# david-cortes/cmfrec

Measured on AMD Instinct MI355X. Metric: ALS rows/sec ((users+items)/iteration time), implicit ALS-CG k=50 fp64, higher is better.
Workload: dtype f64

## Files before the change

cmfrec_amd/csrc/cg_kernels.hpp:

```cpp
#pragma once
#include <hip/hip_runtime.h>
#include <stdint.h>
#include <type_traits>

#include "lanes.hpp"

namespace cmfhip {

constexpr int WAVE = 64;
constexpr int TILE = 64;
constexpr int MAX_W = 8;
#ifndef CMF_CG_WAVES_PER_SIMD
#define CMF_CG_WAVES_PER_SIMD 2
#endif
#ifndef CMF_CG_WAVES_PER_SIMD_F32
#define CMF_CG_WAVES_PER_SIMD_F32 3
#endif
#ifndef CMF_CG_WAVES_PER_SIMD_LOW
#define CMF_CG_WAVES_PER_SIMD_LOW 3
#endif
constexpr int CG_NTSEL_MAX_S = 7;
template <typename T, int W, int NRES_, int NTSEL = 0> constexpr int cg_waves_per_simd()
{
    if (sizeof(T) == 8 && NTSEL == 1 && W <= 8) return CMF_CG_WAVES_PER_SIMD_LOW;
    if (sizeof(T) == 4 && NTSEL == 1 && W <= 4 && NRES_ == 0) return CMF_CG_WAVES_PER_SIMD_F32 + 1;
    return (sizeof(T) == 4 && W <= 4 && NRES_ == 0) ? CMF_CG_WAVES_PER_SIMD_F32 : CMF_CG_WAVES_PER_SIMD;
}
constexpr int CG_NT_LOW = 6;
#ifndef CMF_CG_NT_F32
#define CMF_CG_NT_F32 1
#endif
#ifndef CMF_CG_NT_MIN_S
#define CMF_CG_NT_MIN_S 4
#endif

struct RowDesc {
    int row;
    int nnz;
    unsigned long long st;
};

constexpr int CG_NCOUNTERS = 64;
constexpr int CG_COUNTER_STRIDE = 32;

template <typename T>
__device__ __forceinline__ T cg_div(T num, T den)
{
#ifndef CMF_CG_IEEE_DIV
    if constexpr (sizeof(T) == 4) return num * __builtin_amdgcn_rcpf(den);
    else {
        double y = __builtin_amdgcn_rcp(den);
        double e = __builtin_fma(-den, y, 1.0);
        y = __builtin_fma(y, e, y);
        e = __builtin_fma(-den, y, 1.0);
        y = __builtin_fma(y, e, y);
        double q = num * y;
        const double r = __builtin_fma(-den, q, num);
        return __builtin_fma(r, y, q);
    }
#else
    return num / den;
#endif
}

template <typename V>
__device__ __forceinline__ V lds_g(const V *p) { return *p; }

template <typename T>
struct CgParams {
    T *A;
    size_t lda;
    const T *B;
    size_t ldb;
    int k;
    const size_t *indptr;
    const int *indices;
    const T *values;
    const T *bias_sub;
    const T *weights = nullptr;
    const T *wsum = nullptr;
    const int *order;
    const RowDesc *desc;
    int nrows;
    const T *BtB;
    T lam, lam_last;
    int scale_lam, scale_bias_const;
    int max_cg_steps;
    int precond;
    int koff = 0, kc = 0;
    const T *CtC = nullptr;
    const T *UC = nullptr;
    T w_side = 0;
    int rows_with_u = 0;
    int row_first = 0;
    const size_t *indptr2 = nullptr;
    const int *indices2 = nullptr;
    const T *values2 = nullptr;
    const T *C2 = nullptr;
    int *counter = nullptr;
    int p_side = 0, scale_lam_sideinfo = 0;
    const T *Bi = nullptr;
    const T *BiTBi = nullptr;
    int ki = 0;
    T w_imp = 0;
    const T *rconst = nullptr;
    size_t ldr = 0;
    int gx = 0;
#ifdef CMF_CG_DEBUG
    int dbg = 0;
#endif
#ifdef CMF_CG_TICKS
    unsigned long long *ticks = nullptr;
#endif
};
#ifdef CMF_CG_TICKS
#define CMF_TICK() __builtin_amdgcn_s_memtime()
__device__ __forceinline__ void cg_ticks_flush(unsigned long long *t, int slot, unsigned long long wait, unsigned long long pass, unsigned long long rows,
                                               unsigned long long total, int lane)
{
    if (t != nullptr && lane == 0) {
        atomicAdd(t + 4 * slot + 0, wait); atomicAdd(t + 4 * slot + 1, pass); atomicAdd(t + 4 * slot + 2, rows); atomicAdd(t + 4 * slot + 3, total);
    }
}
#endif
#ifdef CMF_CG_DEBUG
#define CMF_DBG(P, bit) (((P).dbg & (bit)) != 0)
#else
#define CMF_DBG(P, bit) false
#endif
template <int NT, int S, typename TILE, typename T>
__device__ __forceinline__ void dbg_fill_tile(TILE &tile, T val)
{
#pragma unroll
    for (int t = 0; t < NT; t++)
#pragma unroll
        for (int s = 0; s < S; s++) tile.set(t, s, val);
}

template <typename T>
__device__ __forceinline__ T wave_sum(T v) { return lanes::wave_sum(v); }

template <typename T, int NT, int I>
__device__ __forceinline__ T treduce8_low_first(const T (&v)[8], bool h)
{
    if constexpr (I + 4 < NT) {
        T keep = h ? v[I + 4] : v[I];
        return keep + lanes::recv_xor4(v[I], v[I + 4]);
    } else return v[I] + lanes::xor4_lower(v[I]);
}
template <typename T, int NT = 8>
__device__ __forceinline__ T treduce8_low(const T (&v)[8], int lane)
{
    static_assert(NT >= 4 && NT <= 8, "entries per lane group");
    T u[4], q[2];
    bool h = (lane & 4) != 0;
    u[0] = treduce8_low_first<T, NT, 0>(v, h); u[1] = treduce8_low_first<T, NT, 1>(v, h);
    u[2] = treduce8_low_first<T, NT, 2>(v, h); u[3] = treduce8_low_first<T, NT, 3>(v, h);
    h = (lane & 2) != 0;
#pragma unroll
    for (int i = 0; i < 2; i++) {
        T keep = h ? u[i + 2] : u[i];
        T send = h ? u[i] : u[i + 2];
        q[i] = keep + lanes::xor2(send);
    }
    h = (lane & 1) != 0;
    T keep = h ? q[1] : q[0];
    T send = h ? q[0] : q[1];
    return keep + lanes::xor1(send);
}

template <typename T>
__device__ __forceinline__ T treduce8_high(const T (&v)[8], int lane)
{
    T u[4], q[2];
#pragma unroll
    for (int i = 0; i < 4; i++) u[i] = lanes::tswap32_add(v[i], v[i + 4]);
#pragma unroll
    for (int i = 0; i < 2; i++) q[i] = lanes::tswap16_add(u[i], u[i + 2]);
    const bool h = (lane & 8) != 0;
    T keep = h ? q[1] : q[0];
    return keep + lanes::recv_xor8(q[0], q[1]);
}

#ifndef CMF_PASS_VECTOR_LDS
#define CMF_PASS_VECTOR_LDS 2
#endif
template <typename T> constexpr bool pass_vector_in_lds() { return CMF_PASS_VECTOR_LDS == 1 || (CMF_PASS_VECTOR_LDS == 2 && sizeof(T) == 8); }
template <typename T, int S>
__device__ __forceinline__ void replicate(T vdist, T (&vrep)[S], int lane);
template <typename T, int S, int GR = 8>
__device__ __forceinline__ void pass_vector_lds(T vdist, T (&vrep)[S], T (&wts)[8], int lane, T *__restrict__ pv)
{
    const int jj = lane >> 3, ll = lane & 7;
    pv[lane] = vdist;
    __builtin_amdgcn_wave_barrier();
#pragma unroll
    for (int s = 0; s < S; s++) vrep[s] = pv[ll + 8 * s];
    const T *wp = pv + GR * jj;
#pragma unroll
    for (int t = 0; t < GR; t++) wts[t] = wp[t];
    __builtin_amdgcn_wave_barrier();
}

__host__ __device__ constexpr int gram_ld(int S) { return 8 * S + 1; }
#ifndef CMF_GRAM_ROWS_BY_K
#define CMF_GRAM_ROWS_BY_K 1
#endif
template <typename T> __host__ __device__ constexpr int gram_rows(int S) { return (CMF_GRAM_ROWS_BY_K && pass_vector_in_lds<T>()) ? S : 8; }
__host__ __device__ constexpr int gram_ld_rows(int S, int GR)
{
    if (GR == 8) return gram_ld(S);
    int ld = 8 * S;
    while ((S * ld) % 32 != 8 && (S * ld) % 32 != 24) ld++;
    return ld;
}
__host__ __device__ constexpr int gram_ld2(int S) { return 8 * S + 2; }
template <typename T> __host__ __device__ constexpr int gram_elems(int S) { return sizeof(T) == 4 ? 64 * gram_ld2(S) : 64 * gram_ld(S); }
template <typename T, int S, int GR = 8> __device__ __forceinline__ int gram_index(int r, int c)
{
    if constexpr (sizeof(T) == 4) return 2 * ((r >> 1) * gram_ld2(S) + c) + (r & 1);
    else return r * gram_ld_rows(S, GR) + c;
}
template <typename T, int S, int GR = 8>
__device__ __forceinline__ void stage_gramian(T *__restrict__ G, const T *__restrict__ BtB, int k, int tid, int nthreads)
{
    static_assert(GR == 8 || sizeof(T) == 8, "rows by k: double precision");
    for (int e = tid; e < 8 * GR * 8 * S; e += nthreads) {
        const int r = e / (8 * S), c = e % (8 * S);
        G[gram_index<T, S, GR>(r, c)] = (r < k && c < k) ? BtB[(size_t)r * k + c] : T(0);
    }
}

template <typename T, int S>
struct RegTile {
    T v[8][S];
    __device__ __forceinline__ void set(int t, int s, T x) { v[t][s] = x; }
};
typedef float f32x2 __attribute__((ext_vector_type(2)));
template <int S>
struct RegTile<float, S> {
    f32x2 v[4][S];
    __device__ __forceinline__ void set(int t, int s, float x) { v[t >> 1][s][t & 1] = x; }
};

template <typename T>
struct PassAcc {
    T v[8];
    __device__ __forceinline__ void zero()
    {
#pragma unroll
        for (int s = 0; s < 8; s++) v[s] = T(0);
    }
    __device__ __forceinline__ void close(T (&out)[8]) const
    {
#pragma unroll
        for (int s = 0; s < 8; s++) out[s] = v[s];
    }
};
template <>
struct PassAcc<float> {
    f32x2 v[8];
    __device__ __forceinline__ void zero()
    {
#pragma unroll
        for (int s = 0; s < 8; s++) v[s] = f32x2{0.f, 0.f};
    }
    __device__ __forceinline__ void close(float (&out)[8]) const
    {
#pragma unroll
        for (int s = 0; s < 8; s++) out[s] = v[s][0] + v[s][1];
    }
};

#ifndef CMF_CG_EARLY_GATHER
#define CMF_CG_EARLY_GATHER 0
#endif
struct NoAfter {
    template <typename TAG> __device__ __forceinline__ void operator()(TAG) const {}
};
template <int S, typename ACC>
__device__ __forceinline__ void pin_acc(ACC &out)
{
#pragma unroll
    for (int s = 0; s < S; s++) asm volatile("" : "+v"(out.v[s]));
}
template <int TS, typename T, int S, typename TILE>
__device__ __forceinline__ void load_tile_slot(TILE &tile, const char *base, unsigned ldb_bytes, unsigned it, int col_last)
{
    const T *rp = reinterpret_cast<const T *>(base + (unsigned long long)it * ldb_bytes);
#pragma unroll
    for (int s = 0; s < S; s++) tile.set(TS, s, rp[(s < S - 1) ? 8 * s : col_last]);
}

template <typename T, int S, int NT = 8>
__device__ __forceinline__ void load_tile(RegTile<T, S> &tile, const T *__restrict__ Bm, size_t ldb,
                                          int k, int my_idx, int cnt, int lane)
{
    const int jj = lane >> 3, ll = lane & 7;
    int its[8];
    its[0] = lanes::bcast8<0>(my_idx); its[1] = lanes::bcast8<1>(my_idx); its[2] = lanes::bcast8<2>(my_idx);
    its[3] = lanes::bcast8<3>(my_idx);
    if (NT > 4) its[4] = lanes::bcast8<4>(my_idx);
    if (NT > 5) its[5] = lanes::bcast8<5>(my_idx);
    if (NT > 6) its[6] = lanes::bcast8<6>(my_idx);
    if (NT > 7) its[7] = lanes::bcast8<7>(my_idx);
    const int first_idx = __builtin_amdgcn_readfirstlane(my_idx);
    const int col_last = min(ll + 8 * (S - 1), k - 1) - ll;
    const char *base = reinterpret_cast<const char *>(Bm + ll);
    const unsigned ldb_bytes = (unsigned)(ldb * sizeof(T));
#pragma unroll
    for (int t = 0; t < NT; t++) {
        const unsigned it = (unsigned)(((jj * NT + t) < cnt) ? its[t] : first_idx);
        const T *rp = reinterpret_cast<const T *>(base + (unsigned long long)it * ldb_bytes);
#pragma unroll
        for (int s = 0; s < S; s++) tile.set(t, s, rp[(s < S - 1) ? 8 * s : col_last]);
    }
}

template <typename T, bool IMPLICIT, int MODE>
__device__ __forceinline__ T pass_weight(T coef, T x, bool valid, T g = T(1))
{
    T w;
    if (IMPLICIT) {
        if (MODE == 0) w = -(coef - T(1)) * x - coef;
        else           w = coef * (x - T(1)) + coef;
    } else {
        if (MODE == 0) w = -((coef - x) * g);
        else           w = coef * g;
    }
    return valid ? w : T(0);
}

template <typename T>
__device__ __forceinline__ T row_lam_mult(const CgParams<T> &P, int row, int nnz)
{
    return (P.wsum != nullptr) ? P.wsum[row] : (T)nnz;
}
template <typename T, bool IMPLICIT>
__device__ __forceinline__ T entry_weight(const CgParams<T> &P, size_t pos)
{
    if (IMPLICIT) return T(1);
    return (P.weights != nullptr) ? P.weights[pos] : T(1);
}

template <int S, bool IMPLICIT, int MODE, int NT = 8, bool INIT = false, typename AFTER = NoAfter>
__device__ __forceinline__ void tile_pass_f32(const RegTile<float, S> &tile, const float (&vrep)[S], float x, bool valid,
                                          PassAcc<float> &out, int lane, float g = 1.f, AFTER after = AFTER())
{
    static_assert(NT % 2 == 0, "single precision: the entries of a lane group travel in pairs");
    float c[8];
#pragma unroll
    for (int q = 0; q < NT / 2; q++) {
        f32x2 acc = f32x2{0.f, 0.f};
#pragma unroll
        for (int s = 0; s < S; s++) acc += tile.v[q][s] * f32x2{vrep[s], vrep[s]};
        c[2 * q] = acc[0]; c[2 * q + 1] = acc[1];
    }
    float coef = treduce8_low<float, NT>(c, lane);
    const float w = pass_weight<float, IMPLICIT, MODE>(coef, x, valid, g);
    float wts[8];
    wts[0] = lanes::bcast8<0>(w); wts[1] = lanes::bcast8<1>(w); wts[2] = lanes::bcast8<2>(w); wts[3] = lanes::bcast8<3>(w);
    if (NT > 4) { wts[4] = lanes::bcast8<4>(w); wts[5] = lanes::bcast8<5>(w); }
    if (NT > 6) { wts[6] = lanes::bcast8<6>(w); wts[7] = lanes::bcast8<7>(w); }
    if constexpr (std::is_same<AFTER, NoAfter>::value) {
#pragma unroll
    for (int q = 0; q < NT / 2; q++) {
        const f32x2 w2 = f32x2{wts[2 * q], wts[2 * q + 1]};
#pragma unroll
        for (int s = 0; s < S; s++) out.v[s] = (INIT && q == 0) ? w2 * tile.v[q][s] : out.v[s] + w2 * tile.v[q][s];
    }
    } else {
        static_for<0, NT / 2>([&](auto qc) {
            constexpr int q = decltype(qc)::value;
            const f32x2 w2 = f32x2{wts[2 * q], wts[2 * q + 1]};
#pragma unroll
            for (int s = 0; s < S; s++) out.v[s] = (INIT && q == 0) ? w2 * tile.v[q][s] : out.v[s] + w2 * tile.v[q][s];
            pin_acc<S>(out);
            after(std::integral_constant<int, 2 * q>{});
            after(std::integral_constant<int, 2 * q + 1>{});
        });
    }
    if constexpr (INIT) {
#pragma unroll
        for (int s = S; s < 8; s++) out.v[s] = f32x2{0.f, 0.f};
    }
}

template <typename T, int S, bool IMPLICIT, int MODE, int NT = 8, bool INIT = false, typename AFTER = NoAfter>
__device__ __forceinline__ void tile_pass(const RegTile<T, S> &tile, const T (&vrep)[S], T x, bool valid,
                                          PassAcc<T> &out, int lane, T g = T(1), AFTER after = AFTER())
{
    if constexpr (std::is_same<T, float>::value) {
        tile_pass_f32<S, IMPLICIT, MODE, NT, INIT, AFTER>(tile, vrep, x, valid, out, lane, g, after);
    } else {
    T c[8];
// ... 71 lines not shown
    constexpr int LD = gram_ld_rows(S, GR);
    const int jj = lane >> 3, ll = lane & 7;
    if constexpr (std::is_same<T, float>::value && W <= 4) {
#pragma unroll
        for (int q = 0; q < 4; q++) {
            if (W > 1 && (q % W) != wr) continue;
            const f32x2 *g = reinterpret_cast<const f32x2 *>(G) + (jj * 4 + q) * gram_ld2(S) + ll;
            const f32x2 w2 = f32x2{wts[2 * q], wts[2 * q + 1]};
#pragma unroll
            for (int s = 0; s < S; s++) out.v[s] = NEG ? out.v[s] - w2 * lds_g(g + 8 * s) : out.v[s] + w2 * lds_g(g + 8 * s);
        }
    } else {
#pragma unroll
        for (int t = 0; t < GR; t++) {
            if (W > 1 && (t % W) != wr) continue;
#pragma unroll
            for (int s = 0; s < S; s++) {
                if constexpr (std::is_same<T, float>::value) {
                    const float g = G[gram_index<T, S>(jj * 8 + t, ll + 8 * s)];
                    out.v[s][0] = NEG ? out.v[s][0] - wts[t] * g : out.v[s][0] + wts[t] * g;
                } else {
                    const T g = lds_g(G + (jj * GR + t) * LD + ll + 8 * s);
                    out.v[s] = NEG ? out.v[s] - wts[t] * g : out.v[s] + wts[t] * g;
                }
            }
        }
    }
}

template <typename T, int S>
__device__ __forceinline__ void replicate(T vdist, T (&vrep)[S], int lane)
{
    const int ll = lane & 7;
#pragma unroll
    for (int s = 0; s < S; s++) vrep[s] = __shfl(vdist, s * 8 + ll);
}

template <typename T, int S, bool IMPLICIT, int W, int RPB, bool GRAMX = false, int NRES_ = 0, int NTSEL = 0>
__global__ void __launch_bounds__(64 * W * RPB, (cg_waves_per_simd<T, W, NRES_, NTSEL>()))
cg_rows_kernel(const CgParams<T> P)
{
    constexpr bool GRAM = IMPLICIT || GRAMX;
    extern __shared__ __attribute__((aligned(16))) unsigned char smem_raw[];
    T *G = reinterpret_cast<T *>(smem_raw);
    T *red = G + (GRAM ? gram_elems<T>(S) : 0);
    const int tid = threadIdx.x;
    const int lane = tid & 63;
    const int wave = tid >> 6;
    const int grp = wave / W;
    const int wr = wave % W;
    const int k = P.k;

    const int nteams = gridDim.x * RPB;
    __shared__ int s_claim[4];
    constexpr bool PV = pass_vector_in_lds<T>();
    __shared__ __attribute__((aligned(16))) T s_pv[PV ? W * RPB : 1][PV ? 64 : 1];
    const int cslot = (blockIdx.x * RPB + grp) % CG_NCOUNTERS;
    int *const my_counter = P.counter + cslot * CG_COUNTER_STRIDE;
    const int cbase = nteams + cslot;
    auto issue_claim = [&]() -> int {
        int v = 0;
        if (wr == 0 && lane == 0) v = atomicAdd(my_counter, 1);
        return v;
    };
    int rnxt, rnn;
    if (W == 1) {
        const int c1 = issue_claim(), c2 = issue_claim();
        rnxt = cbase + CG_NCOUNTERS * __builtin_amdgcn_readfirstlane(c1);
        rnn = cbase + CG_NCOUNTERS * __builtin_amdgcn_readfirstlane(c2);
    } else if (wr == 0 && lane == 0) {
        s_claim[2] = cbase + CG_NCOUNTERS * atomicAdd(my_counter, 1);
        s_claim[3] = cbase + CG_NCOUNTERS * atomicAdd(my_counter, 1);
    }
    constexpr int GR = gram_rows<T>(S);
    if (GRAM) stage_gramian<T, S, GR>(G, P.BtB, k, tid, blockDim.x);
    if (GRAM || W > 1) __syncthreads();
    if (W > 1) { rnxt = s_claim[2]; rnn = s_claim[3]; }
    T *myred = red + (size_t)grp * 2 * W * 64;

    int buf = 0;
    static_assert(W == 1 || RPB == 1, "multi-wave teams own their workgroup (barriers are per row)");

    constexpr int NRES = NRES_ > 0 ? NRES_ : ((std::is_same<T, float>::value && W == 8) ? 2 : 1);
    static_assert(NRES == 1 || std::is_same<T, float>::value, "two resident tiles: single precision");
    static_assert(NTSEL == 0 || (S >= CMF_CG_NT_MIN_S && (sizeof(T) == 4 || S <= CG_NTSEL_MAX_S) && NRES_ == 0),
                  "launches by tile size: tiles by row length (double precision: k <= 56)");
    constexpr int NT_MIN = (S >= CMF_CG_NT_MIN_S && (CMF_CG_NT_F32 || !std::is_same<T, float>::value)) ? (std::is_same<T, float>::value ? 6 : 5) : 8;
    auto nt_of = [&](int nnz_) -> int {
        int nt = (nnz_ + 8 * W * NRES - 1) / (8 * W * NRES);
        if (std::is_same<T, float>::value) nt = (nt + 1) & ~1;
        return (nt > 8) ? 8 : (nt < NT_MIN ? NT_MIN : nt);
    };
    struct Pre { int idx; T x; T a; int idx2; T x2; T g; T g2; };
    auto load_desc = [&](int rix_) -> RowDesc {
        RowDesc d; d.row = 0; d.nnz = 0; d.st = 0;
        if (rix_ < P.nrows) d = P.desc[rix_];
        d.row = __builtin_amdgcn_readfirstlane(d.row);
        d.nnz = __builtin_amdgcn_readfirstlane(d.nnz);
        d.st = ((unsigned long long)(unsigned)__builtin_amdgcn_readfirstlane((int)(d.st >> 32)) << 32) |
               (unsigned)__builtin_amdgcn_readfirstlane((int)(d.st & 0xffffffffu));
        return d;
    };
    auto load_pre = [&](const RowDesc &d) -> Pre {
        Pre q; q.idx = 0; q.x = T(0); q.a = T(0); q.idx2 = 0; q.x2 = T(0); q.g = T(1); q.g2 = T(1);
        const int nt = nt_of(d.nnz), tl = 8 * nt;
        const int b = lane & 7;
        const int ent = (lane >> 3) * nt + b;
        const int cnt = min(tl, d.nnz - wr * tl);
        if (b < nt && ent < cnt) {
            const size_t pos = d.st + (size_t)wr * tl + ent;
            q.idx = P.indices[pos];
            q.x = P.values[pos];
            q.g = entry_weight<T, IMPLICIT>(P, pos);
            if (!IMPLICIT && P.bias_sub != nullptr) q.x -= P.bias_sub[q.idx];
        }
        if (NRES == 2) {
            const int cnt2 = min(tl, d.nnz - (wr + W) * tl);
            if (b < nt && ent < cnt2) {
                const size_t pos = d.st + (size_t)(wr + W) * tl + ent;
                q.idx2 = P.indices[pos];
                q.x2 = P.values[pos];
                q.g2 = entry_weight<T, IMPLICIT>(P, pos);
                if (!IMPLICIT && P.bias_sub != nullptr) q.x2 -= P.bias_sub[q.idx2];
            }
        }
        if (d.nnz > 0 && lane < k) q.a = P.A[(size_t)d.row * P.lda + lane];
        return q;
    };
    int rix = blockIdx.x * RPB + grp;
    RowDesc dcur = load_desc(rix);
    RowDesc dnxt = load_desc(rnxt);
    Pre pcur = load_pre(dcur);
    int pend = issue_claim();
    constexpr bool EARLY = CMF_CG_EARLY_GATHER != 0;
    constexpr int NT_MAX = (NTSEL == 1) ? CG_NT_LOW : 8;
    RegTile<T, S> tile_c;
    RegTile<T, (NRES == 2) ? S : 1> tile2_c;
    const char *const gbase = reinterpret_cast<const char *>(P.B + (lane & 7));
    const unsigned gldb = (unsigned)(P.ldb * sizeof(T));
    const int gcol_last = min((lane & 7) + 8 * (S - 1), k - 1) - (lane & 7);
    auto gather_slot = [&](auto &tl_, auto tc, int idx_, int first_idx_, int nt_, int cnt_) {
        constexpr int t = decltype(tc)::value;
        if constexpr (t < NT_MAX) {
            if (t < nt_) {
                const unsigned it_ = (unsigned)((((lane >> 3) * nt_ + t) < cnt_) ? lanes::bcast8<t>(idx_) : first_idx_);
                load_tile_slot<t, T, S>(tl_, gbase, gldb, it_, gcol_last);
            }
        }
    };
    struct Want { int nt0, cnt0, nt1, cnt1; };
    auto want_of = [&](const RowDesc &d) -> Want {
        Want w_;
        const int nt = nt_of(d.nnz), tl = 8 * nt;
        w_.cnt0 = min(tl, d.nnz - wr * tl);
        w_.nt0 = (w_.cnt0 > 0 && !CMF_DBG(P, 1)) ? nt : 0;
        w_.cnt1 = (NRES == 2) ? min(tl, d.nnz - (wr + W) * tl) : 0;
        w_.nt1 = (w_.cnt1 > 0 && !CMF_DBG(P, 1)) ? nt : 0;
        return w_;
    };
    auto gather_row = [&](const RowDesc &d, const Pre &q) {
        const Want w_ = want_of(d);
        const int f0 = __builtin_amdgcn_readfirstlane(q.idx);
        static_for<0, NT_MAX>([&](auto tc) { gather_slot(tile_c, tc, q.idx, f0, w_.nt0, w_.cnt0); });
        if constexpr (NRES == 2) {
            const int f1 = __builtin_amdgcn_readfirstlane(q.idx2);
            static_for<0, NT_MAX>([&](auto tc) { gather_slot(tile2_c, tc, q.idx2, f1, w_.nt1, w_.cnt1); });
        }
    };
    if constexpr (EARLY) gather_row(dcur, pcur);
#ifdef CMF_CG_TICKS
    unsigned long long tk_wait = 0, tk_pass = 0, tk_rows = 0;
    const unsigned long long tk_begin = CMF_TICK();
#endif
    int it = 0;
    RowDesc dnn;
    Pre pnxt;
    auto solve_row = [&](auto nt_tag) {
        constexpr int NT = decltype(nt_tag)::value;
        constexpr int TL = 8 * NT;
        const int row = dcur.row;
        const size_t st = dcur.st;
        const int nnz = dcur.nnz;
        const int ntiles = (nnz + TL - 1) / TL;
        const int my_ntiles = (ntiles > wr) ? (ntiles - wr + W - 1) / W : 0;
        const bool resident = NT < 8 || my_ntiles <= NRES;

        T lam = P.lam, lam_last = P.lam_last;
        if (GRAMX && P.kc > 0) {
            if (P.scale_lam || P.scale_lam_sideinfo) {
                T mult = row_lam_mult(P, row, nnz);
                if (P.scale_lam_sideinfo) mult += (T)P.p_side;
                lam *= mult; lam_last *= mult;
            }
        } else if (!IMPLICIT && P.scale_lam) {
            const T mult = row_lam_mult(P, row, nnz);
            lam *= mult;
            if (!P.scale_bias_const) lam_last *= mult;
        }
        T *arow = P.A + (size_t)row * P.lda;
        T a_d = pcur.a;

        RegTile<T, S> tile_r;
        RegTile<T, (NRES == 2) ? S : 1> tile2_r;
        auto &tile = [&]() -> RegTile<T, S> & { if constexpr (EARLY) return tile_c; else return tile_r; }();
        auto &tile2 = [&]() -> RegTile<T, (NRES == 2) ? S : 1> & { if constexpr (EARLY) return tile2_c; else return tile2_r; }();
        const int ent = (lane >> 3) * NT + (lane & 7);
        const bool lane_has = (NT == 8) || (lane & 7) < NT;
        const int cnt0 = min(TL, nnz - wr * TL);
        T x_res = pcur.x;
        const T g_res = pcur.g;
        bool valid_res = lane_has && ent < cnt0;
        if (CMF_DBG(P, 1)) dbg_fill_tile<8, S>(tile, (T)(pcur.idx & 3) * (T)0.001);
        else if (!EARLY && cnt0 > 0) load_tile<T, S, NT>(tile, P.B, P.ldb, k, pcur.idx, cnt0, lane);
        const int cnt1 = (NRES == 2) ? min(TL, nnz - (wr + W) * TL) : 0;
        const T x2_res = pcur.x2, g2_res = pcur.g2;
        const bool valid2_res = lane_has && ent < cnt1;
        if constexpr (NRES == 2) {
            if (!EARLY && cnt1 > 0 && !CMF_DBG(P, 1)) load_tile<T, S, NT>(tile2, P.B, P.ldb, k, pcur.idx2, cnt1, lane);
        }
        dnn = load_desc(rnn);
        pnxt = load_pre(dnxt);
#ifdef CMF_CG_TICKS
        const unsigned long long tk0 = CMF_TICK();
        asm volatile("s_waitcnt vmcnt(0)" ::: "memory");
        const unsigned long long tk1 = CMF_TICK();
        tk_wait += tk1 - tk0;
#endif

        auto run_pass = [&](T vdist, auto mode_tag, bool first, auto fin_tag) -> T {
            constexpr int MODE = decltype(mode_tag)::value;
            constexpr bool FIN = decltype(fin_tag)::value && EARLY;
            asm volatile("" ::: "memory");
            T vrep[S];
            T gw[8];
            if constexpr (PV) pass_vector_lds<T, S, GR>(vdist, vrep, gw, lane, &s_pv[wave][0]);
            else replicate<T, S>(vdist, vrep, lane);
            PassAcc<T> acc;
            acc.zero();
            if constexpr (FIN) {
                if (NT < 8 || NRES == 2 || resident) {
                    const Want nx = want_of(dnxt);
                    const int f0 = __builtin_amdgcn_readfirstlane(pnxt.idx);
                    auto after0 = [&](auto tc) { gather_slot(tile, tc, pnxt.idx, f0, nx.nt0, nx.cnt0); };
                    if (cnt0 > 0 && !CMF_DBG(P, 4)) {
                        tile_pass<T, S, IMPLICIT, MODE, NT>(tile, vrep, x_res, valid_res, acc, lane, g_res, after0);
                        static_for<NT, NT_MAX>(after0);
                    } else static_for<0, NT_MAX>(after0);
                    if constexpr (NRES == 2) {
                        const int f1 = __builtin_amdgcn_readfirstlane(pnxt.idx2);
                        auto after1 = [&](auto tc) { gather_slot(tile2, tc, pnxt.idx2, f1, nx.nt1, nx.cnt1); };
                        if (cnt1 > 0 && !CMF_DBG(P, 4)) {
                            tile_pass<T, S, IMPLICIT, MODE, NT>(tile2, vrep, x2_res, valid2_res, acc, lane, g2_res, after1);
                            static_for<NT, NT_MAX>(after1);
                        } else static_for<0, NT_MAX>(after1);
                    }
                } else {
                for (int tl = wr; tl < ntiles; tl += W) {
                    const int cnt = min(TL, nnz - tl * TL);
                    const bool valid = lane_has && ent < cnt;
                    const size_t pos = st + (size_t)tl * TL + ent;
                    int my_idx = valid ? P.indices[pos] : 0;
                    T x = valid ? P.values[pos] : T(0);
                    const T g = valid ? entry_weight<T, IMPLICIT>(P, pos) : T(1);
                    if (!IMPLICIT && P.bias_sub != nullptr && valid) x -= P.bias_sub[my_idx];
                    if (!CMF_DBG(P, 1)) load_tile<T, S, NT>(tile, P.B, P.ldb, k, my_idx, cnt, lane);
                    if (!CMF_DBG(P, 4)) tile_pass<T, S, IMPLICIT, MODE, NT>(tile, vrep, x, valid, acc, lane, g);
                }
                gather_row(dnxt, pnxt);
                }
            } else
            if constexpr (NRES == 2) {
                if (cnt0 > 0 && !CMF_DBG(P, 4)) tile_pass<T, S, IMPLICIT, MODE, NT>(tile, vrep, x_res, valid_res, acc, lane, g_res);
                if (cnt1 > 0 && !CMF_DBG(P, 4)) tile_pass<T, S, IMPLICIT, MODE, NT>(tile2, vrep, x2_res, valid2_res, acc, lane, g2_res);
            } else if constexpr (NT < 8) {
                if (cnt0 > 0 && !CMF_DBG(P, 4)) tile_pass<T, S, IMPLICIT, MODE, NT>(tile, vrep, x_res, valid_res, acc, lane, g_res);
            } else
            for (int tl = wr; tl < ntiles; tl += W) {
                T x, g; bool valid;
                const bool have = (tl == wr) && (resident || first);
                if (!have) {
                    const int cnt = min(TL, nnz - tl * TL);
                    valid = lane_has && ent < cnt;
                    const size_t pos = st + (size_t)tl * TL + ent;
                    int my_idx = valid ? P.indices[pos] : 0;
                    x = valid ? P.values[pos] : T(0);
                    g = valid ? entry_weight<T, IMPLICIT>(P, pos) : T(1);
                    if (!IMPLICIT && P.bias_sub != nullptr && valid) x -= P.bias_sub[my_idx];
                    if (!CMF_DBG(P, 1)) load_tile<T, S, NT>(tile, P.B, P.ldb, k, my_idx, cnt, lane);
                } else {
                    x = x_res; g = g_res; valid = valid_res;
                }
                if (!CMF_DBG(P, 4)) tile_pass<T, S, IMPLICIT, MODE, NT>(tile, vrep, x, valid, acc, lane, g);
            }
            if (GRAM && !CMF_DBG(P, 2)) {
                if constexpr (PV) gram_pass_w<MODE == 0, T, S, W, GR>(G, gw, acc, lane, wr);
                else gram_pass<T, S, W>(G, (MODE == 0) ? -vdist : vdist, acc, lane, wr);
            }
            T out[8];
            acc.close(out);
            T tot = treduce8_high<T>(out, lane);
            if (W > 1) {
                T *rb = myred + (size_t)buf * W * 64;
                rb[wr * 64 + lane] = tot;
                if (first && wr == 0 && lane == 0) s_claim[it & 1] = cbase + CG_NCOUNTERS * pend;
                __syncthreads();
                tot = T(0);
#pragma unroll
                for (int w = 0; w < W; w++) tot += rb[w * 64 + lane];
                buf ^= 1;
            }
            return tot;
        };

        T r_d = run_pass(a_d, std::integral_constant<int, 0>{}, true, std::false_type{});
        r_d -= lam * a_d;
        if (!IMPLICIT && lam != lam_last && lane == k - 1) r_d -= (lam_last - lam) * a_d;
        if (GRAMX && P.rconst != nullptr && lane < k) r_d += P.rconst[(size_t)row * P.ldr + lane];
        if (lane >= k) r_d = T(0);
        T p_d = r_d;
        T r_old = CMF_DBG(P, 8) ? T(1) : wave_sum(r_d * r_d);
        bool done = (r_old <= (T)1e-12);
        for (int step = 0; step < P.max_cg_steps - (EARLY ? 1 : 0) && !done; step++) {
            T Ap_d = run_pass(p_d, std::integral_constant<int, 1>{}, false, std::false_type{});
            Ap_d += lam * p_d;
            if (!IMPLICIT && lam != lam_last && lane == k - 1) Ap_d += (lam_last - lam) * p_d;
            if (lane >= k) Ap_d = T(0);
            T alpha = CMF_DBG(P, 8) ? T(0.001) : cg_div(r_old, wave_sum(Ap_d * p_d));
            a_d += alpha * p_d;
            if (!EARLY && step == P.max_cg_steps - 1) break;
            r_d -= alpha * Ap_d;
            T r_new = CMF_DBG(P, 8) ? T(0.5) : wave_sum(r_d * r_d);
            if (r_new <= (T)1e-8) done = true;
            else {
                p_d = p_d * cg_div(r_new, r_old) + r_d;
                r_old = r_new;
            }
        }
        if (EARLY && P.max_cg_steps > 0 && !done) {
            T Ap_d = run_pass(p_d, std::integral_constant<int, 1>{}, false, std::true_type{});
            Ap_d += lam * p_d;
            if (!IMPLICIT && lam != lam_last && lane == k - 1) Ap_d += (lam_last - lam) * p_d;
            if (lane >= k) Ap_d = T(0);
            const T alpha = CMF_DBG(P, 8) ? T(0.001) : cg_div(r_old, wave_sum(Ap_d * p_d));
            a_d += alpha * p_d;
        } else if constexpr (EARLY) gather_row(dnxt, pnxt);
#ifdef CMF_CG_TICKS
        tk_pass += CMF_TICK() - tk1; tk_rows += (wr == 0);
#endif
        if (wr == 0 && lane < k) arow[lane] = a_d;
    };
    for (; rix < P.nrows; it++) {
        const int nt = nt_of(dcur.nnz);
        if constexpr (NT_MIN == 8) solve_row(std::integral_constant<int, 8>{});
        else if constexpr (std::is_same<T, float>::value) {
            if constexpr (NTSEL == 1) solve_row(std::integral_constant<int, 6>{});
            else if constexpr (NTSEL == 2) solve_row(std::integral_constant<int, 8>{});
            else if (nt == 6) solve_row(std::integral_constant<int, 6>{});
            else solve_row(std::integral_constant<int, 8>{});
        } else if constexpr (NTSEL == 1) {
            if (nt <= 5) solve_row(std::integral_constant<int, 5>{});
            else solve_row(std::integral_constant<int, 6>{});
        } else if constexpr (NTSEL == 2) {
            if (nt <= 7) solve_row(std::integral_constant<int, 7>{});
            else solve_row(std::integral_constant<int, 8>{});
        } else {
            switch (nt) {
                case 5: solve_row(std::integral_constant<int, 5>{}); break;
                case 6: solve_row(std::integral_constant<int, 6>{}); break;
                case 7: solve_row(std::integral_constant<int, 7>{}); break;
                default: solve_row(std::integral_constant<int, 8>{}); break;
            }
        }
        const int r3 = (W == 1) ? cbase + CG_NCOUNTERS * __builtin_amdgcn_readfirstlane(pend) : s_claim[it & 1];
        dcur = dnxt; dnxt = dnn; pcur = pnxt;
        rix = rnxt; rnxt = rnn; rnn = r3;
        pend = issue_claim();
    }
// ... 1017 lines not shown
```

cmfrec_amd/csrc/device.hpp:

```cpp
#pragma once
#include <hip/hip_runtime.h>
#include <algorithm>
#include <cstdio>
#include <cstdlib>
#include <cstring>
#include <numeric>
#include <string>
#include <vector>

#include "../../include/cmfrec_hip.h"
#include "device_base.hpp"
#include "cg_kernels.hpp"
#include "chol_kernels.hpp"
#include "dense_kernels.hpp"
#include "gram_cg_kernels.hpp"
#include "topn_kernels.hpp"

namespace cmfhip {

constexpr int MAX_DEVICES = 16;
constexpr int NBINS = 6;
constexpr int BIN_VHEAVY = 0;
constexpr int BIN_HEAVY = 1;
constexpr int BIN_MED4 = 2;
// ... 546 lines not shown
    EventPair ev{nullptr, nullptr};
    if (tm) {
        HIP_CHECK(hipEventCreate(&ev.a));
        HIP_CHECK(hipEventCreate(&ev.b));
        HIP_CHECK(hipEventRecord(ev.a, dev.stream));
    }
    if (vh_takes_gram<GRAMX>(P.k, X)) {
        GramParams<real_t> G;
        G.sl_vrow = X.sl_vrow.ptr; G.sl_first = X.sl_first.ptr; G.sl_count = X.sl_count.ptr; G.row_sl_off = X.row_sl_off.ptr;
        G.part = X.gram_part.ptr; G.n_slices = X.n_slices; G.nvh = nvh;
        P.nrows = nvh;
#ifdef CMF_CG_DEBUG
        if (switches().debug_ticks) {
            static unsigned long long *d_t = nullptr;
            unsigned long long h[4];
            if (d_t == nullptr) { HIP_CHECK(hipMalloc((void **)&d_t, sizeof(h))); HIP_CHECK(hipMemset(d_t, 0, sizeof(h))); }
            else {
                HIP_CHECK(hipDeviceSynchronize());
                HIP_CHECK(hipMemcpy(h, d_t, sizeof(h), hipMemcpyDeviceToHost));
                if (h[1] > 0)
                    fprintf(stderr, "gram_wave: %.0f ticks per wave, %llu waves, %llu slices, %llu nnz: %.1f ticks per nnz and wave\n",
                            (double)h[0] / h[1], h[1], h[2], h[3], (double)h[0] / (double)h[3]);
                HIP_CHECK(hipMemset(d_t, 0, sizeof(h)));
            }
            G.ticks = d_t;
        }
#endif
        poison_lds(dev.stream, dev.num_cus);
        const bool slice_kernel = switches().gram_slice;
        if (slice_kernel)
            hipLaunchKernelGGL((gram_slice_kernel<real_t, IMPLICIT>), dim3(std::min(X.n_slices, dev.num_cus * 2)), dim3(64 * GRAM_NW), 0,
                           dev.stream, P, G);
        else {
            const dim3 gw(std::min((X.n_slices + 3) / 4, dev.num_cus * 4));
            const int rem = (sizeof(real_t) == 8) ? P.k - 16 * (GRAM_NTT - 1) : 0;
            launch_gram_wave(gw, dev.stream, P, G, IMPLICIT, rem);
        }
        poison_lds(dev.stream, dev.num_cus);
        hipLaunchKernelGGL((gram_cg_kernel<real_t, IMPLICIT>), dim3(std::min(nvh, dev.num_cus * 8)), dim3(256), 0, dev.stream, P, G);
        HIP_CHECK(hipGetLastError());
        if (tm) {
            HIP_CHECK(hipEventRecord(ev.b, dev.stream));
            tm->ev[BIN_VHEAVY].push_back(ev);
        }
        return;
    }
    VhState<real_t> V;
    V.r = X.vh_r.ptr; V.p = X.vh_p.ptr; V.r_old = X.vh_r_old.ptr; V.done = X.vh_done.ptr; V.part = X.vh_part.ptr;
    V.chunk_row = X.vh_chunk_row.ptr; V.chunk_start = X.vh_chunk_start.ptr; V.chunk_cnt = X.vh_chunk_cnt.ptr;
    V.chunk_off = X.vh_chunk_off.ptr; V.launch = X.vh_launch.ptr; V.work = X.vh_work.ptr;
    V.nvh = nvh; V.nchunks = X.n_chunks; V.nlaunch = X.n_launch;
    P.nrows = nvh;
    poison_lds(dev.stream, dev.num_cus);
    const dim3 gp(X.n_launch), bp(64 * VH_CHUNK_TILES), gu(nvh), bu(64 * VH_UPD_WAVES);
    hipLaunchKernelGGL((vh_pass_kernel<real_t, S, IMPLICIT, 0>), gp, bp, 0, dev.stream, P, V);
    hipLaunchKernelGGL((vh_update_kernel<real_t, IMPLICIT, 0, GRAMX>), gu, bu, 0, dev.stream, P, V);
    for (int step = 0; step < P.max_cg_steps; step++) {
        hipLaunchKernelGGL((vh_pass_kernel<real_t, S, IMPLICIT, 1>), gp, bp, 0, dev.stream, P, V);
        hipLaunchKernelGGL((vh_update_kernel<real_t, IMPLICIT, 1, GRAMX>), gu, bu, 0, dev.stream, P, V);
    }
    HIP_CHECK(hipGetLastError());
    if (tm) {
        HIP_CHECK(hipEventRecord(ev.b, dev.stream));
        tm->ev[BIN_VHEAVY].push_back(ev);
    }
}

inline int cg_bin_streams()
{
    const int n = switches().bins_par;
    return std::min(std::max(n, 1), DeviceInfo::MAX_BIN_STREAMS + 1);
}

template <int S, bool IMPLICIT, int W, int RPB, bool GRAMX>
inline void launch_cg_bin_by_tile(const DeviceInfo &dev, const CgParams<real_t> &P, const SparseShard &X, int first, int count, BinTimers *tm, int bin,
                                  hipStream_t st)
{
#ifdef CMFREC_HIP_FLOAT
    constexpr bool by_tile = S >= CMF_CG_NT_MIN_S && CMF_CG_NT_F32 && W <= 4;
#else
    constexpr bool by_tile = S >= CMF_CG_NT_MIN_S && S <= CG_NTSEL_MAX_S && (W == 1 || W == 4 || W == 8);
#endif
    if (count <= 0) return;
    if constexpr (by_tile) {
        if (switches().nt_split) {
            const int n_hi = std::min(count, std::max(0, X.n_gt_low[W == 1 ? 0 : W == 2 ? 1 : W == 4 ? 2 : 3] - first));
            EventPair ev{nullptr, nullptr};
            if (tm) { HIP_CHECK(hipEventCreate(&ev.a)); HIP_CHECK(hipEventCreate(&ev.b)); HIP_CHECK(hipEventRecord(ev.a, st)); }
            launch_cg_bin<S, IMPLICIT, W, RPB, GRAMX, 0, 2>(dev, P, first, n_hi, nullptr, bin, st);
            launch_cg_bin<S, IMPLICIT, W, RPB, GRAMX, 0, 1>(dev, P, first + n_hi, count - n_hi, nullptr, bin, st, NBINS + 2 + bin);
            if (tm) { HIP_CHECK(hipEventRecord(ev.b, st)); tm->ev[bin].push_back(ev); }
            return;
        }
    }
    launch_cg_bin<S, IMPLICIT, W, RPB, GRAMX>(dev, P, first, count, tm, bin, st);
}

template <int S, bool IMPLICIT, bool GRAMX>
inline void launch_cg_any_bin(const DeviceInfo &dev, const CgParams<real_t> &P, const SparseShard &X, BinTimers *tm, int bin, hipStream_t st)
{
    const int first = X.bin_first[bin], count = X.bin_rows[bin];
    switch (bin) {
        case BIN_HEAVY:
#ifdef CMFREC_HIP_FLOAT
            {
                const int n_long8 = std::min(count, std::max(0, X.n_gt512 - first));
                EventPair ev{nullptr, nullptr};
                if (tm) { HIP_CHECK(hipEventCreate(&ev.a)); HIP_CHECK(hipEventCreate(&ev.b)); HIP_CHECK(hipEventRecord(ev.a, st)); }
                launch_cg_bin<S, IMPLICIT, 8, 1, GRAMX>(dev, P, first, n_long8, nullptr, bin, st);
                launch_cg_bin<S, IMPLICIT, 4, 1, GRAMX, 2>(dev, P, first + n_long8, count - n_long8, nullptr, bin, st, NBINS);
                if (tm) { HIP_CHECK(hipEventRecord(ev.b, st)); tm->ev[bin].push_back(ev); }
                break;
            }
#endif
            launch_cg_bin_by_tile<S, IMPLICIT, 8, 1, GRAMX>(dev, P, X, first, count, tm, bin, st); break;
        case BIN_MED4: launch_cg_bin_by_tile<S, IMPLICIT, 4, 1, GRAMX>(dev, P, X, first, count, tm, bin, st); break;
        case BIN_MED2: launch_cg_bin_by_tile<S, IMPLICIT, 2, 1, GRAMX>(dev, P, X, first, count, tm, bin, st); break;
        default: launch_cg_bin_by_tile<S, IMPLICIT, 1, 4, GRAMX>(dev, P, X, first, count, tm, bin, st); break;
    }
}

template <int S, bool IMPLICIT, bool GRAMX = false>
inline void launch_cg_S(const DeviceInfo &dev, const CgParams<real_t> &P, const SparseShard &X, BinTimers *tm)
{
    if (dev.row_counter.n < ROW_COUNTER_INTS) const_cast<DeviceInfo &>(dev).row_counter.alloc(ROW_COUNTER_INTS);
    HIP_CHECK(hipMemsetAsync(dev.row_counter.ptr, 0, ROW_COUNTER_INTS * sizeof(int), dev.stream));
    const bool vh_aside = X.bin_rows[BIN_VHEAVY] > 0 && X.vh_runs_aside(dev.num_cus) && !vh_takes_gram<GRAMX>(P.k, X);
    const bool alt = X.is_part;
    DeviceInfo &d = const_cast<DeviceInfo &>(dev);
    const int npar = cg_bin_streams();
    if (npar > 1 && !(vh_aside || alt)) {
        d.ensure_bin_streams(npar - 1);
        hipStream_t ss[DeviceInfo::MAX_BIN_STREAMS + 1];
        ss[0] = dev.stream;
        for (int i = 1; i < npar; i++) ss[i] = d.bin_streams[i - 1];
        HIP_CHECK(hipEventRecord(d.fork_ev, dev.stream));
        for (int i = 1; i < npar; i++) HIP_CHECK(hipStreamWaitEvent(ss[i], d.fork_ev, 0));
        static const double row_equiv[NBINS] = {0.0, 126.0, 7.0, 7.0, 0.0, 11.5};
        double cost[NBINS], load[DeviceInfo::MAX_BIN_STREAMS + 1] = {0, 0, 0, 0, 0, 0};
        int order_b[NBINS];
        for (int b = 0; b < NBINS; b++) {
            cost[b] = (double)X.bin_nnz[b] + row_equiv[b] * (double)X.bin_rows[b];
            order_b[b] = b;
        }
        std::sort(order_b, order_b + NBINS, [&](int a, int b2) { return cost[a] > cost[b2]; });
        for (int q = 0; q < NBINS; q++) {
            const int b = order_b[q];
            if (X.bin_rows[b] <= 0) continue;
            int si = 0;
            for (int i = 1; i < npar; i++) if (load[i] < load[si]) si = i;
            load[si] += cost[b];
            if (b == BIN_VHEAVY) launch_cg_vheavy<S, IMPLICIT, GRAMX>(dev, P, X, tm, ss[si]);
            else if (b == BIN_TINY) launch_cg_tiny<S, IMPLICIT, GRAMX>(dev, P, X.bin_first[BIN_TINY], X.bin_rows[BIN_TINY], tm, ss[si], X.n_gt16);
            else launch_cg_any_bin<S, IMPLICIT, GRAMX>(dev, P, X, tm, b, ss[si]);
        }
        for (int i = 1; i < npar; i++) {
            HIP_CHECK(hipEventRecord(d.bin_join[i - 1], ss[i]));
            HIP_CHECK(hipStreamWaitEvent(dev.stream, d.bin_join[i - 1], 0));
        }
        return;
    }
    if (vh_aside || alt) {
        d.ensure_aux();
        HIP_CHECK(hipEventRecord(d.fork_ev, dev.stream));
        HIP_CHECK(hipStreamWaitEvent(d.aux_stream, d.fork_ev, 0));
    }
// ... 186 lines not shown
```

cmfrec_amd/csrc/device_base.hpp:

```cpp
#pragma once
#include <hip/hip_runtime.h>
#include <cstdio>
#include <cstdlib>
#include <cstring>
#include <functional>
#include <new>
#include <string>

#include "../../include/cmfrec_hip.h"

namespace cmfhip {

extern thread_local std::string g_last_error;
extern thread_local int g_last_rc;

struct HipError {
    int code;
};

inline void hip_check(hipError_t e, const char *what, const char *file, int line)
{
    if (e == hipSuccess) return;
    char buf[512];
    snprintf(buf, sizeof buf, "cmfrec_hip: %s failed: %s (%s:%d)", what, hipGetErrorString(e), file, line);
    g_last_error = buf;
    fprintf(stderr, "%s\n", buf);
    throw HipError{e == hipErrorOutOfMemory ? 1 : 4};
}
#define HIP_CHECK(x) ::cmfhip::hip_check((x), #x, __FILE__, __LINE__)

inline int guarded(const std::function<int()> &f)
{
    try {
        return f();
    } catch (const HipError &e) {
        return e.code;
    } catch (const std::bad_alloc &) {
        g_last_error = "cmfrec_hip: host out of memory";
        return 1;
    }
}

struct Switches {
    bool poison_lds = false;
    int vh_min = 0;
    int vh = 0;
    bool gram_slice = false;
    int bins_par = 2;
    bool nt_split = true;
    bool cg_generic = false;
    int chol = 0;
    int parts_coop = 1;
    int chol_wg = 2;
    int gramk = -1;
    int gramk_batch = 0;
    int lowrank = -1;
    bool topn_wide = false;
    int topn_tiles = 0;
    int topn_cand_waves = 0;
    int rank_slice = 0;
    bool eig_jacobi = false;
    int debug_skip = 0;
    bool debug_ticks = false;
    int cg_teams = 0;
    int newrows_block_rows = 0;
    int predict_block = 0;
    void reload()
    {
        auto str = [](const char *n) -> const char * { const char *v = getenv(n); return (v != nullptr && v[0] != 0) ? v : nullptr; };
        auto num = [&](const char *n, int dflt) -> int { const char *v = str(n); return v ? atoi(v) : dflt; };
        poison_lds = str("CMFREC_HIP_POISON_LDS") != nullptr;
        vh_min = num("CMFREC_HIP_VH_MIN", 0);
        const char *v = str("CMFREC_HIP_VH");
        vh = !v ? 0 : strcmp(v, "stream") == 0 ? 1 : strcmp(v, "gram") == 0 ? 2 : 1;
        v = str("CMFREC_HIP_GRAM_KERNEL"); gram_slice = v && strcmp(v, "slice") == 0;
        bins_par = num("CMFREC_HIP_BINS_PAR", 2);
        nt_split = num("CMFREC_HIP_NT_SPLIT", 1) != 0;
        v = str("CMFREC_HIP_CG_KERNEL"); cg_generic = v && strcmp(v, "generic") == 0;
        v = str("CMFREC_HIP_CHOL"); chol = !v ? 0 : strcmp(v, "rows") == 0 ? 1 : strcmp(v, "noslices") == 0 ? 2 : 0;
        parts_coop = num("CMFREC_HIP_PARTS_COOP", 1);
        chol_wg = num("CMFREC_HIP_CHOL_WG", 2);
        if (chol_wg == 1) chol_wg = 2;
        gramk = num("CMFREC_HIP_GRAMK", -1);
        gramk_batch = num("CMFREC_HIP_GRAMK_BATCH", 0);
        lowrank = num("CMFREC_HIP_LOWRANK", -1);
        v = str("CMFREC_HIP_TOPN"); topn_wide = v && strcmp(v, "wide") == 0;
        topn_tiles = num("CMFREC_HIP_TOPN_TILES", 0);
        topn_cand_waves = num("CMFREC_HIP_TOPN_CAND_WAVES", 0);
        rank_slice = num("CMFREC_HIP_RANK_SLICE", 0);
        v = str("CMFREC_HIP_EIG"); eig_jacobi = v && strcmp(v, "jacobi") == 0;
        debug_skip = num("CMFREC_HIP_CG_SKIP", num("CMFREC_HIP_CHOL_SKIP", num("CMFREC_HIP_WAVE_SKIP", 0)));
        debug_ticks = str("CMFREC_HIP_GRAM_TICKS") != nullptr || str("CMFREC_HIP_CHOL_TICKS") != nullptr;
        cg_teams = num("CMFREC_HIP_CG_TEAMS", 0);
        newrows_block_rows = num("CMFREC_HIP_NEWROWS_BLOCK_ROWS", 0);
        predict_block = num("CMFREC_HIP_PREDICT_BLOCK", 0);
    }
};
inline Switches &switches_mut() { static Switches sw; static bool first = (sw.reload(), true); (void)first; return sw; }
inline const Switches &switches() { return switches_mut(); }

template <typename T>
struct DevBuf {
    T *ptr = nullptr;
    size_t n = 0;
    bool owned = true;
    DevBuf() = default;
    DevBuf(const DevBuf &) = delete;
    DevBuf &operator=(const DevBuf &) = delete;
    ~DevBuf() { release(); }
    void release()
    {
        if (ptr && owned) (void)hipFree(ptr);
        ptr = nullptr;
        n = 0;
    }
    void alloc(size_t count)
    {
        release();
        n = count;
        owned = true;
        if (count) HIP_CHECK(hipMalloc((void **)&ptr, count * sizeof(T)));
        if (count && switches().poison_lds) {
            HIP_CHECK(hipMemset(ptr, 0xFF, count * sizeof(T)));
            HIP_CHECK(hipDeviceSynchronize());
        }
    }
    void alloc_at_least(size_t count)
    {
        if (n < count) alloc(count);
    }
    void upload(const T *host, size_t count, hipStream_t st)
    {
        if (count > n) alloc(count);
        if (count) HIP_CHECK(hipMemcpyAsync(ptr, host, count * sizeof(T), hipMemcpyDefault, st));
    }
    void download(T *host, size_t count, hipStream_t st) const
    {
        if (count) HIP_CHECK(hipMemcpyAsync(host, ptr, count * sizeof(T), hipMemcpyDeviceToHost, st));
    }
};

inline void upload_columns(real_t *dst, size_t dld, const real_t *src, size_t ld, size_t rows, size_t cols, hipStream_t st)
{
    if (ld == cols && dld == cols) HIP_CHECK(hipMemcpyAsync(dst, src, rows * cols * sizeof(real_t), hipMemcpyDefault, st));
    else HIP_CHECK(hipMemcpy2DAsync(dst, dld * sizeof(real_t), src, ld * sizeof(real_t), cols * sizeof(real_t), rows, hipMemcpyDefault, st));
}

struct DeviceScope {
    int prev = -1;
    explicit DeviceScope(int device)
    {
        int cur = -1;
        HIP_CHECK(hipGetDevice(&cur));
        if (cur != device) { HIP_CHECK(hipSetDevice(device)); prev = cur; }
    }
    ~DeviceScope() { if (prev >= 0) (void)hipSetDevice(prev); }
};

void open_device(int device, int *device_id, int *num_cus, hipStream_t *stream);

// ... 2 lines not shown
```

Measured before the change: 170.6 million.

## Launch low-fill fp64 CG rows on half-width teams holding two resident tiles

For double precision, rows in the low-fill bins of the 2- and 8-wave CG launches now go to a half-width team where each wave holds two register tiles (NRES=2), at 2 waves per SIMD. Value, weight and A-row loads are deferred until after the B-tile gathers are issued. The gramian weight read from LDS is moved to right before the gram pass. The aim is fewer idle lanes and waves for short rows, and better overlap of gather latency. The cost is higher register pressure and lower occupancy for those launches, plus an extra kernel launch per bin. A new env switch controls the path and defaults to on.

```diff
diff --git a/cmfrec_amd/csrc/cg_kernels.hpp b/cmfrec_amd/csrc/cg_kernels.hpp
--- a/cmfrec_amd/csrc/cg_kernels.hpp
+++ b/cmfrec_amd/csrc/cg_kernels.hpp
@@ -22,6 +22,7 @@
 constexpr int CG_NTSEL_MAX_S = 7;
 template <typename T, int W, int NRES_, int NTSEL = 0> constexpr int cg_waves_per_simd()
 {
+    if (sizeof(T) == 8 && NTSEL == 1 && NRES_ == 2) return 2;
     if (sizeof(T) == 8 && NTSEL == 1 && W <= 8) return CMF_CG_WAVES_PER_SIMD_LOW;
     if (sizeof(T) == 4 && NTSEL == 1 && W <= 4 && NRES_ == 0) return CMF_CG_WAVES_PER_SIMD_F32 + 1;
     return (sizeof(T) == 4 && W <= 4 && NRES_ == 0) ? CMF_CG_WAVES_PER_SIMD_F32 : CMF_CG_WAVES_PER_SIMD;
@@ -188,7 +189,7 @@
 template <typename T> constexpr bool pass_vector_in_lds() { return CMF_PASS_VECTOR_LDS == 1 || (CMF_PASS_VECTOR_LDS == 2 && sizeof(T) == 8); }
 template <typename T, int S>
 __device__ __forceinline__ void replicate(T vdist, T (&vrep)[S], int lane);
-template <typename T, int S, int GR = 8>
+template <typename T, int S, int GR = 8, bool WTS = true>
 __device__ __forceinline__ void pass_vector_lds(T vdist, T (&vrep)[S], T (&wts)[8], int lane, T *__restrict__ pv)
 {
     const int jj = lane >> 3, ll = lane & 7;
@@ -196,7 +197,18 @@
     __builtin_amdgcn_wave_barrier();
 #pragma unroll
     for (int s = 0; s < S; s++) vrep[s] = pv[ll + 8 * s];
-    const T *wp = pv + GR * jj;
+    if constexpr (WTS) {
+        const T *wp = pv + GR * jj;
+#pragma unroll
+        for (int t = 0; t < GR; t++) wts[t] = wp[t];
+    }
+    __builtin_amdgcn_wave_barrier();
+}
+template <typename T, int GR>
+__device__ __forceinline__ void pass_vector_lds_weights(T (&wts)[8], int lane, const T *__restrict__ pv)
+{
+    asm volatile("" ::: "memory");
+    const T *wp = pv + GR * (lane >> 3);
 #pragma unroll
     for (int t = 0; t < GR; t++) wts[t] = wp[t];
     __builtin_amdgcn_wave_barrier();
@@ -292,7 +304,7 @@
     for (int s = 0; s < S; s++) tile.set(TS, s, rp[(s < S - 1) ? 8 * s : col_last]);
 }
 
-template <typename T, int S, int NT = 8>
+template <typename T, int S, int NT = 8, bool UCMP = false>
 __device__ __forceinline__ void load_tile(RegTile<T, S> &tile, const T *__restrict__ Bm, size_t ldb,
                                           int k, int my_idx, int cnt, int lane)
 {
@@ -308,9 +320,11 @@
     const int col_last = min(ll + 8 * (S - 1), k - 1) - ll;
     const char *base = reinterpret_cast<const char *>(Bm + ll);
     const unsigned ldb_bytes = (unsigned)(ldb * sizeof(T));
+    const int slots_in = cnt - jj * NT;
 #pragma unroll
     for (int t = 0; t < NT; t++) {
-        const unsigned it = (unsigned)(((jj * NT + t) < cnt) ? its[t] : first_idx);
+        const bool in_tile = UCMP ? (t < slots_in) : ((jj * NT + t) < cnt);
+        const unsigned it = (unsigned)(in_tile ? its[t] : first_idx);
         const T *rp = reinterpret_cast<const T *>(base + (unsigned long long)it * ldb_bytes);
 #pragma unroll
         for (int s = 0; s < S; s++) tile.set(t, s, rp[(s < S - 1) ? 8 * s : col_last]);
@@ -548,8 +562,10 @@
     static_assert(W == 1 || RPB == 1, "multi-wave teams own their workgroup (barriers are per row)");
 
     constexpr int NRES = NRES_ > 0 ? NRES_ : ((std::is_same<T, float>::value && W == 8) ? 2 : 1);
-    static_assert(NRES == 1 || std::is_same<T, float>::value, "two resident tiles: single precision");
-    static_assert(NTSEL == 0 || (S >= CMF_CG_NT_MIN_S && (sizeof(T) == 4 || S <= CG_NTSEL_MAX_S) && NRES_ == 0),
+    static_assert(NRES == 1 || std::is_same<T, float>::value || NTSEL == 1,
+                  "two resident tiles: single precision, or the double-precision launch of 5 / 6 entries per lane group");
+    static_assert(NTSEL == 0 || (S >= CMF_CG_NT_MIN_S && (sizeof(T) == 4 || S <= CG_NTSEL_MAX_S) &&
+                                 (NRES_ == 0 || (sizeof(T) == 8 && NTSEL == 1 && NRES_ == 2))),
                   "launches by tile size: tiles by row length (double precision: k <= 56)");
     constexpr int NT_MIN = (S >= CMF_CG_NT_MIN_S && (CMF_CG_NT_F32 || !std::is_same<T, float>::value)) ? (std::is_same<T, float>::value ? 6 : 5) : 8;
     auto nt_of = [&](int nnz_) -> int {
@@ -558,6 +574,7 @@
         return (nt > 8) ? 8 : (nt < NT_MIN ? NT_MIN : nt);
     };
     struct Pre { int idx; T x; T a; int idx2; T x2; T g; T g2; };
+    constexpr bool LATEV = NRES == 2 && sizeof(T) == 8;
     auto load_desc = [&](int rix_) -> RowDesc {
         RowDesc d; d.row = 0; d.nnz = 0; d.st = 0;
         if (rix_ < P.nrows) d = P.desc[rix_];
@@ -576,22 +593,46 @@
         if (b < nt && ent < cnt) {
             const size_t pos = d.st + (size_t)wr * tl + ent;
             q.idx = P.indices[pos];
-            q.x = P.values[pos];
-            q.g = entry_weight<T, IMPLICIT>(P, pos);
-            if (!IMPLICIT && P.bias_sub != nullptr) q.x -= P.bias_sub[q.idx];
+            if constexpr (!LATEV) {
+                q.x = P.values[pos];
+                q.g = entry_weight<T, IMPLICIT>(P, pos);
+                if (!IMPLICIT && P.bias_sub != nullptr) q.x -= P.bias_sub[q.idx];
+            }
         }
         if (NRES == 2) {
             const int cnt2 = min(tl, d.nnz - (wr + W) * tl);
             if (b < nt && ent < cnt2) {
                 const size_t pos = d.st + (size_t)(wr + W) * tl + ent;
                 q.idx2 = P.indices[pos];
-                q.x2 = P.values[pos];
-                q.g2 = entry_weight<T, IMPLICIT>(P, pos);
-                if (!IMPLICIT && P.bias_sub != nullptr) q.x2 -= P.bias_sub[q.idx2];
-            }
+                if constexpr (!LATEV) {
+                    q.x2 = P.values[pos];
+                    q.g2 = entry_weight<T, IMPLICIT>(P, pos);
+                    if (!IMPLICIT && P.bias_sub != nullptr) q.x2 -= P.bias_sub[q.idx2];
+                }
+            }
+        }
+        if constexpr (!LATEV) {
+            if (d.nnz > 0 && lane < k) q.a = P.A[(size_t)d.row * P.lda + lane];
+        }
+        return q;
+    };
+    auto load_pre_values = [&](const RowDesc &d, Pre &q) {
+        const int nt = nt_of(d.nnz), tl = 8 * nt;
+        const int b = lane & 7;
+        const int ent = (lane >> 3) * nt + b;
+        if (b < nt && ent < min(tl, d.nnz - wr * tl)) {
+            const size_t pos = d.st + (size_t)wr * tl + ent;
+            q.x = P.values[pos];
+            q.g = entry_weight<T, IMPLICIT>(P, pos);
+            if (!IMPLICIT && P.bias_sub != nullptr) q.x -= P.bias_sub[q.idx];
+        }
+        if (b < nt && ent < min(tl, d.nnz - (wr + W) * tl)) {
+            const size_t pos = d.st + (size_t)(wr + W) * tl + ent;
+            q.x2 = P.values[pos];
+            q.g2 = entry_weight<T, IMPLICIT>(P, pos);
+            if (!IMPLICIT && P.bias_sub != nullptr) q.x2 -= P.bias_sub[q.idx2];
         }
         if (d.nnz > 0 && lane < k) q.a = P.A[(size_t)d.row * P.lda + lane];
-        return q;
     };
     int rix = blockIdx.x * RPB + grp;
     RowDesc dcur = load_desc(rix);
@@ -674,15 +715,19 @@
         const bool lane_has = (NT == 8) || (lane & 7) < NT;
         const int cnt0 = min(TL, nnz - wr * TL);
         T x_res = pcur.x;
-        const T g_res = pcur.g;
+        T g_res = pcur.g;
         bool valid_res = lane_has && ent < cnt0;
         if (CMF_DBG(P, 1)) dbg_fill_tile<8, S>(tile, (T)(pcur.idx & 3) * (T)0.001);
-        else if (!EARLY && cnt0 > 0) load_tile<T, S, NT>(tile, P.B, P.ldb, k, pcur.idx, cnt0, lane);
+        else if (!EARLY && cnt0 > 0) load_tile<T, S, NT, LATEV>(tile, P.B, P.ldb, k, pcur.idx, cnt0, lane);
         const int cnt1 = (NRES == 2) ? min(TL, nnz - (wr + W) * TL) : 0;
-        const T x2_res = pcur.x2, g2_res = pcur.g2;
+        T x2_res = pcur.x2, g2_res = pcur.g2;
         const bool valid2_res = lane_has && ent < cnt1;
         if constexpr (NRES == 2) {
-            if (!EARLY && cnt1 > 0 && !CMF_DBG(P, 1)) load_tile<T, S, NT>(tile2, P.B, P.ldb, k, pcur.idx2, cnt1, lane);
+            if (!EARLY && cnt1 > 0 && !CMF_DBG(P, 1)) load_tile<T, S, NT, LATEV>(tile2, P.B, P.ldb, k, pcur.idx2, cnt1, lane);
+        }
+        if constexpr (LATEV) {
+            load_pre_values(dcur, pcur);
+            a_d = pcur.a; x_res = pcur.x; g_res = pcur.g; x2_res = pcur.x2; g2_res = pcur.g2;
         }
         dnn = load_desc(rnn);
         pnxt = load_pre(dnxt);
@@ -699,7 +744,7 @@
             asm volatile("" ::: "memory");
             T vrep[S];
             T gw[8];
-            if constexpr (PV) pass_vector_lds<T, S, GR>(vdist, vrep, gw, lane, &s_pv[wave][0]);
+            if constexpr (PV) pass_vector_lds<T, S, GR, !(LATEV && GRAM)>(vdist, vrep, gw, lane, &s_pv[wave][0]);
             else replicate<T, S>(vdist, vrep, lane);
             PassAcc<T> acc;
             acc.zero();
@@ -759,6 +804,7 @@
                 if (!CMF_DBG(P, 4)) tile_pass<T, S, IMPLICIT, MODE, NT>(tile, vrep, x, valid, acc, lane, g);
             }
             if (GRAM && !CMF_DBG(P, 2)) {
+                if constexpr (PV && LATEV) pass_vector_lds_weights<T, GR>(gw, lane, &s_pv[wave][0]);
                 if constexpr (PV) gram_pass_w<MODE == 0, T, S, W, GR>(G, gw, acc, lane, wr);
                 else gram_pass<T, S, W>(G, (MODE == 0) ? -vdist : vdist, acc, lane, wr);
             }
diff --git a/cmfrec_amd/csrc/device.hpp b/cmfrec_amd/csrc/device.hpp
--- a/cmfrec_amd/csrc/device.hpp
+++ b/cmfrec_amd/csrc/device.hpp
@@ -652,6 +652,22 @@
     constexpr bool by_tile = S >= CMF_CG_NT_MIN_S && S <= CG_NTSEL_MAX_S && (W == 1 || W == 4 || W == 8);
 #endif
     if (count <= 0) return;
+#ifndef CMFREC_HIP_FLOAT
+    constexpr bool two_tiles = S >= CMF_CG_NT_MIN_S && S <= CG_NTSEL_MAX_S && (W == 2 || W == 8) && RPB == 1 && !(GRAMX && S == CG_NTSEL_MAX_S);
+    if constexpr (two_tiles) {
+        const int tt = switches().two_tiles;
+        if (tt == 1 || tt == (W == 2 ? 2 : 3)) {
+            const int n_hi = std::min(count, std::max(0, X.n_gt_low[W == 2 ? 1 : 3] - first));
+            EventPair ev{nullptr, nullptr};
+            if (tm) { HIP_CHECK(hipEventCreate(&ev.a)); HIP_CHECK(hipEventCreate(&ev.b)); HIP_CHECK(hipEventRecord(ev.a, st)); }
+            if (switches().nt_split) launch_cg_bin<S, IMPLICIT, W, 1, GRAMX, 0, 2>(dev, P, first, n_hi, nullptr, bin, st);
+            else launch_cg_bin<S, IMPLICIT, W, 1, GRAMX>(dev, P, first, n_hi, nullptr, bin, st);
+            launch_cg_bin<S, IMPLICIT, W / 2, (W == 2) ? 4 : 1, GRAMX, 2, 1>(dev, P, first + n_hi, count - n_hi, nullptr, bin, st, NBINS + 2 + bin);
+            if (tm) { HIP_CHECK(hipEventRecord(ev.b, st)); tm->ev[bin].push_back(ev); }
+            return;
+        }
+    }
+#endif
     if constexpr (by_tile) {
         if (switches().nt_split) {
             const int n_hi = std::min(count, std::max(0, X.n_gt_low[W == 1 ? 0 : W == 2 ? 1 : W == 4 ? 2 : 3] - first));
diff --git a/cmfrec_amd/csrc/device_base.hpp b/cmfrec_amd/csrc/device_base.hpp
--- a/cmfrec_amd/csrc/device_base.hpp
+++ b/cmfrec_amd/csrc/device_base.hpp
@@ -48,6 +48,7 @@
     bool gram_slice = false;
     int bins_par = 2;
     bool nt_split = true;
+    int two_tiles = 1;
     bool cg_generic = false;
     int chol = 0;
     int parts_coop = 1;
@@ -76,6 +77,7 @@
         v = str("CMFREC_HIP_GRAM_KERNEL"); gram_slice = v && strcmp(v, "slice") == 0;
         bins_par = num("CMFREC_HIP_BINS_PAR", 2);
         nt_split = num("CMFREC_HIP_NT_SPLIT", 1) != 0;
+        two_tiles = num("CMFREC_HIP_TWO_TILES", 1);
         v = str("CMFREC_HIP_CG_KERNEL"); cg_generic = v && strcmp(v, "generic") == 0;
         v = str("CMFREC_HIP_CHOL"); chol = !v ? 0 : strcmp(v, "rows") == 0 ? 1 : strcmp(v, "noslices") == 0 ? 2 : 0;
         parts_coop = num("CMFREC_HIP_PARTS_COOP", 1);
```

Result: faster. 174.9 million, median of 6 (+2.5%).
